# cram9030/continuum-robot

Hardware: AMD Instinct MI355X
Metric: beam-element-steps/s (higher is better)
Workload: dtype f64

## Files before the change

### continuum-robot_amd/csrc/crb_blocked.h

```cpp
#pragma once
#include <cmath>
#include <cstring>
#include <vector>

#include "crb_math.h"

namespace crb {

constexpr int BLK_NPL = 4;
constexpr int BLK_LANES = 64;
constexpr int BLK_S = BLK_NPL * BLK_LANES;
constexpr int BLK_MAX_LV = 6;
constexpr int BLK_PACK = 5;
enum : int {
    BU_L1 = 0, BU_L2 = 5, BU_D0 = 10, BU_D1 = 15, BU_D2 = 20, BU_U0 = 25, BU_U1 = 30,
    BU_WL = 35, BU_WR = 50, BU_AS = 65, BU_CS = 70, BU_N = 76
};
__host__ __device__ constexpr int blk_sep_vals(int levels) { return levels * PCR_LEVEL_VALS + BLK_PACK; }
__host__ __device__ constexpr int blk_fold_offset(int levels) { return BU_N + blk_sep_vals(levels) * BLK_LANES; }

constexpr int BLK_TAB_ROW = 16;
constexpr int BLK_TAB_REGS = (BU_N + BLK_TAB_ROW - 1) / BLK_TAB_ROW;
__host__ __device__ constexpr int blk_tab_index(int reg, int lane) {
    return BLK_TAB_ROW * reg + (lane & (BLK_TAB_ROW - 1)) < BU_N - 1 ? BLK_TAB_ROW * reg + (lane & (BLK_TAB_ROW - 1)) : BU_N - 1;
}

#if defined(__HIPCC__)
template <int OFF, typename T>
__device__ __forceinline__ void blk_bc_fnma(const T (&tab)[BLK_TAB_REGS], T x, T& acc) {
    static_assert(OFF >= 0 && OFF < BU_N, "table offset");
#if defined(__HIP_DEVICE_COMPILE__)
    asm("v_fmac_f64_dpp %0, -%1, %2 row_newbcast:%3 row_mask:0xf bank_mask:0xf"
        : "+v"(acc) : "v"(tab[OFF / BLK_TAB_ROW]), "v"(x), "n"(OFF % BLK_TAB_ROW));
#else
    acc -= tab[OFF / BLK_TAB_ROW] * x;
#endif
}
template <int OFF, typename T>
__device__ __forceinline__ void blk_bc_fma(const T (&tab)[BLK_TAB_REGS], T x, T& acc) {
    static_assert(OFF >= 0 && OFF < BU_N, "table offset");
#if defined(__HIP_DEVICE_COMPILE__)
    asm("v_fmac_f64_dpp %0, %1, %2 row_newbcast:%3 row_mask:0xf bank_mask:0xf"
        : "+v"(acc) : "v"(tab[OFF / BLK_TAB_ROW]), "v"(x), "n"(OFF % BLK_TAB_ROW));
#else
    acc += tab[OFF / BLK_TAB_ROW] * x;
#endif
}
template <int OFF, typename T>
__device__ __forceinline__ T blk_bc_copy(const T (&tab)[BLK_TAB_REGS]) {
    static_assert(OFF >= 0 && OFF < BU_N, "table offset");
#if defined(__HIP_DEVICE_COMPILE__)
    T d;
    asm("v_mov_b64_dpp %0, %1 row_newbcast:%2 row_mask:0xf bank_mask:0xf" : "=v"(d) : "v"(tab[OFF / BLK_TAB_ROW]), "n"(OFF % BLK_TAB_ROW));
    return d;
#else
    return tab[OFF / BLK_TAB_ROW];
#endif
}
template <int OFF, typename T>
__device__ __forceinline__ void blk_bc_sub_mul(const T (&tab)[BLK_TAB_REGS], const T v[3], T o[3]) {
    blk_bc_fnma<OFF + 0>(tab, v[0], o[0]);
    blk_bc_fnma<OFF + 1>(tab, v[1], o[1]);
    blk_bc_fnma<OFF + 2>(tab, v[2], o[1]);
    blk_bc_fnma<OFF + 3>(tab, v[1], o[2]);
    blk_bc_fnma<OFF + 4>(tab, v[2], o[2]);
}
#endif

template <typename T, typename P = const T*>
__host__ __device__ __forceinline__ void blk_mul(P m, const T v[3], T o[3]) {
    o[0] = m[0] * v[0];
    o[1] = m[1] * v[1] + m[2] * v[2];
    o[2] = m[3] * v[1] + m[4] * v[2];
}
template <typename T, typename P = const T*>
__host__ __device__ __forceinline__ void blk_sub_mul(P m, const T v[3], T o[3]) {
    o[0] = o[0] - m[0] * v[0];
    o[1] = o[1] - m[1] * v[1] - m[2] * v[2];
    o[2] = o[2] - m[3] * v[1] - m[4] * v[2];
}
template <typename T, typename P = const T*>
__host__ __device__ __forceinline__ void blk_interior_solve(P u, const T r[][3], T y[3][3]) {
    T z1[3] = {r[1][0], r[1][1], r[1][2]}, z2[3] = {r[2][0], r[2][1], r[2][2]};
    blk_sub_mul<T, P>(u + BU_L1, r[0], z1);
    blk_sub_mul<T, P>(u + BU_L2, z1, z2);
    blk_mul<T, P>(u + BU_D2, z2, y[2]);
    blk_mul<T, P>(u + BU_D1, z1, y[1]);
    blk_sub_mul<T, P>(u + BU_U1, y[2], y[1]);
    blk_mul<T, P>(u + BU_D0, r[0], y[0]);
    blk_sub_mul<T, P>(u + BU_U0, y[1], y[0]);
}

struct Blk2 {
    double ax = 0.0, m[4] = {0.0, 0.0, 0.0, 0.0};
};
inline Blk2 b2_mul(const Blk2& a, const Blk2& b) {
    Blk2 r;
    r.ax = a.ax * b.ax;
    mul2(a.m, b.m, r.m);
    return r;
}
inline Blk2 b2_sub(const Blk2& a, const Blk2& b) {
// ... 159 lines not shown
```

### continuum-robot_amd/csrc/crb_lean.h

```cpp
#pragma once
#include <hip/hip_runtime.h>

#include "crb_blocked.h"
#include "crb_generic.h"

namespace crb {

template <typename T>
struct LeanRec {
    static constexpr int N = sizeof(T) == 8 ? 10 : 12;
    static constexpr int V = 16 / sizeof(T);
};
template <typename T>
__host__ __device__ constexpr size_t lean_lds_bytes(int NT, int lognw) {
    return sizeof(T) * (size_t(NT + 1) * LeanRec<T>::N * (lognw == 1 ? 2 : 1) +
                        (sizeof(T) == 4 ? 4 : 3) * size_t(NT + 1) * size_t(lognw > 1 ? lognw - 1 : 0));
}

__device__ __forceinline__ double dpp_from_lower(double x) {
    int lo = __double2loint(x), hi = __double2hiint(x);
    lo = __builtin_amdgcn_mov_dpp(lo, 0x138, 0xf, 0xf, true);
    hi = __builtin_amdgcn_mov_dpp(hi, 0x138, 0xf, 0xf, true);
    return __hiloint2double(hi, lo);
}
// ... 66 lines not shown
            for (int c = 0; c < 3; ++c) {
                switch (l - LOGNW) {
                    case 0: rlo[c] = lane_lower<T, 1>(r[c], lane); rhi[c] = lane_higher<T, 1>(r[c], lane); break;
                    case 1: rlo[c] = lane_lower<T, 2>(r[c], lane); rhi[c] = lane_higher<T, 2>(r[c], lane); break;
                    case 2: rlo[c] = lane_lower<T, 4>(r[c], lane); rhi[c] = lane_higher<T, 4>(r[c], lane); break;
                    case 3: rlo[c] = lane_lower<T, 8>(r[c], lane); rhi[c] = lane_higher<T, 8>(r[c], lane); break;
                    case 4: rlo[c] = lane_lower<T, 16>(r[c], lane); rhi[c] = lane_higher<T, 16>(r[c], lane); break;
                    default: rlo[c] = lane_lower<T, 32>(r[c], lane); rhi[c] = lane_higher<T, 32>(r[c], lane); break;
                }
            }
            if (ISOLATE) {
                const int st = 1 << l;
                const bool lo_ok = valid && j - st >= 0, hi_ok = valid && j + st < S;
#pragma unroll
                for (int c = 0; c < 3; ++c) { rlo[c] = lo_ok ? rlo[c] : T(0); rhi[c] = hi_ok ? rhi[c] : T(0); }
            }
        }
        pcr_apply_level<T>(cf.lv[l], rlo, rhi, r);
    }
    CRB_SETPRIO(sizeof(T) == 4 ? P32_FIN : P_FIN);
    pcr_apply_final<T>(cf.fin, r, a);
}

template <typename T, int LV, int LOGNW, int EM>
__device__ __forceinline__ void lean_rhs(const ElemCoef<T>& ec, T dragc, bool corrected, const SolveCoef<T, LV>& cf, T* lds3, int t,
                                         int lane, int j, int S, bool valid, const T sq[3], const T sv[3], const T uadd[3], T a[3]) {
    constexpr int NW = 1 << LOGNW, NT = 64 << LOGNW, NULLT = NT;
    T* const ldsQ = lds3;
    T* const ldsA = lds3 + 3 * size_t(NT + 1);
    T* const ldsB = lds3 + 9 * size_t(NT + 1);
    auto thread_of = [](int jj) { return ((jj & (NW - 1)) << 6) | (jj >> LOGNW); };
    const int t_l1 = (valid && j >= 1) ? thread_of(j - 1) : NULLT;
    const int t_r1 = (valid && j + 1 < S) ? thread_of(j + 1) : NULLT;
    const int t_r2 = (valid && j + 2 < S) ? thread_of(j + 2) : NULLT;
    T qL[3];
    if (LOGNW == 0) {
#pragma unroll
        for (int c = 0; c < 3; ++c) qL[c] = lane_lower<T, 1>(sq[c], lane);
    } else {
#pragma unroll
        for (int c = 0; c < 3; ++c) ldsQ[size_t(c) * (NT + 1) + t] = sq[c];
        __syncthreads();
#pragma unroll
        for (int c = 0; c < 3; ++c) qL[c] = ldsQ[size_t(c) * (NT + 1) + t_l1];
    }
    T fl[3], fr[3];
    if (EM == EM_NONLINEAR) elem_force_nonlinear<T>(ec.c, qL, sq, false, fl, fr);
    else if (EM == EM_LINEAR) elem_force_linear<T>(ec.c, qL, sq, fl, fr);
    else elem_force<T>(ec, qL, sq, corrected, fl, fr);
    T pp[3];
#pragma unroll
    for (int c = 0; c < 3; ++c) pp[c] = uadd[c] - fr[c];
    pp[1] += drag_force<T>(dragc, sv[1]);
    T r[3], rlo[3], rhi[3];
    if (LOGNW == 0) {
#pragma unroll
        for (int c = 0; c < 3; ++c) {
            r[c] = pp[c] - lane_higher<T, 1>(fl[c], lane);
            rlo[c] = lane_lower<T, 1>(r[c], lane);
            rhi[c] = lane_higher<T, 1>(r[c], lane);
        }
    } else {
        auto col = [&](int k, int th) -> T& { return ldsA[size_t(k) * (NT + 1) + th]; };
#pragma unroll
        for (int c = 0; c < 3; ++c) { col(c, t) = pp[c]; col(3 + c, t) = fl[c]; }
        __syncthreads();
#pragma unroll
        for (int c = 0; c < 3; ++c) {
            rlo[c] = col(c, t_l1) - fl[c];
            r[c] = pp[c] - col(3 + c, t_r1);
            rhi[c] = col(c, t_r1) - col(3 + c, t_r2);
        }
    }
    pcr_apply_level<T>(cf.lv[0], rlo, rhi, r);
    lean_reduce_tail<T, LV, LOGNW>(cf, ldsB, t, lane, j, S, valid, r, a);
}

#ifndef CRB_BLK_CHORD
#define CRB_BLK_CHORD 1
#endif
#ifndef CRB_BLK_FOLD
#define CRB_BLK_FOLD 1
#endif
#ifndef CRB_BLK_RK4_POS
#define CRB_BLK_RK4_POS 1
#endif
constexpr int BLK_STRIP_PAD = 4;
constexpr int BLK_STRIP_W = BLK_STRIP_PAD + BLK_LANES + BLK_STRIP_PAD;
__host__ __device__ constexpr size_t blk_lds_bytes(int ls) {
    return size_t(blk_sep_vals(ls) + 1) / 2 * 2 * BLK_LANES * sizeof(double) + size_t(4) * 3 * BLK_STRIP_W * sizeof(double);
}
template <typename T, int LS, int EM, typename KPT>
__device__ __forceinline__ void lean_blocked_body(KPT kp) {
    static_assert(sizeof(T) == 8, "the blocked stepper is fp64");
    static_assert(LS == 3 && (1 << (LS - 1)) == BLK_STRIP_PAD, "the strip carries the third separator level, stride 4");
    constexpr int NP = BLK_NPL, NV = blk_sep_vals(LS), NV2 = (NV + 1) / 2;
    constexpr bool REGROUP = EM == EM_NONLINEAR && !CRB_LITERAL_POLY;
    constexpr bool CHORD = CRB_BLK_CHORD, RKPOS = CRB_BLK_RK4_POS;
    constexpr bool FOLD = REGROUP && CRB_BLK_FOLD;
#if defined(__HIP_DEVICE_COMPILE__)
    typedef const __attribute__((address_space(4))) SlotConst<T>* CS;
    typedef const __attribute__((address_space(4))) T* CK;
#define CRB_BFRESH(ptr) asm volatile("" : "+s"(ptr))
#else
    typedef const SlotConst<T>* CS;
    typedef const T* CK;
#define CRB_BFRESH(ptr) (void)(ptr)
#endif
    typedef T rec4 __attribute__((ext_vector_type(4)));
    typedef T pair2 __attribute__((ext_vector_type(2)));
    KParams<T> p = *(const KParams<T>*)(kp);
    extern __shared__ __attribute__((aligned(16))) unsigned char crb_smem[];
    pair2* const sepL = reinterpret_cast<pair2*>(crb_smem);
    T* const strips = reinterpret_cast<T*>(sepL + NV2 * 64);
    const int t = threadIdx.x, lane = t & 63;
    const int wave = __builtin_amdgcn_readfirstlane(t >> 6);
    {
        const T* src = p.blocked + BU_N;
        for (int i = t; i < NV2 * 64; i += 256) {
            const int v = 2 * (i >> 6), l = i & 63;
            sepL[i] = pair2{src[size_t(v) * 64 + l], v + 1 < NV ? src[size_t(v + 1) * 64 + l] : T(0)};
        }
        for (int i = t; i < 4 * 3 * BLK_STRIP_W; i += 256) {
            const int k = i % BLK_STRIP_W;
            if (k < BLK_STRIP_PAD || k >= BLK_STRIP_PAD + BLK_LANES) strips[i] = T(0);
        }
    }
#if defined(__HIP_DEVICE_COMPILE__)
    typedef volatile __attribute__((address_space(3))) T* SP;
#else
    typedef volatile T* SP;
#endif
    const SP strip = (SP)(strips + wave * 3 * BLK_STRIP_W + BLK_STRIP_PAD + lane);
    T tab[BLK_TAB_REGS];
#pragma unroll
    for (int i = 0; i < BLK_TAB_REGS; ++i) tab[i] = p.blocked[blk_tab_index(i, lane)];
    const T cD2[3] = {blk_bc_copy<BU_D2>(tab), blk_bc_copy<BU_D2 + 2>(tab), blk_bc_copy<BU_D2 + 4>(tab)};
    const T cD1[3] = {blk_bc_copy<BU_U1>(tab), blk_bc_copy<BU_D1 + 2>(tab), blk_bc_copy<BU_D1 + 4>(tab)};
    const T cD0[3] = {blk_bc_copy<BU_U0>(tab), blk_bc_copy<BU_D0 + 2>(tab), blk_bc_copy<BU_D0 + 4>(tab)};
    __syncthreads();
    const int n_groups = (p.B + 3) / 4;
    for (int grp = blockIdx.x; grp < n_groups; grp += gridDim.x) {
        CRB_BFRESH(kp);
        p = *(const KParams<T>*)(kp);
        const int beam = grp * 4 + wave;
        if (beam >= p.B) continue;
        const size_t plane = size_t(p.n_node) * 4;
        const size_t xoff = size_t(beam) * 2 * plane + size_t(NP * lane + p.off) * 4;
        T xq[NP][3], xv[NP][3];
#pragma unroll
        for (int k = 0; k < NP; ++k) {
            const rec4 a = *reinterpret_cast<const rec4*>(p.x + xoff + 4 * k), b = *reinterpret_cast<const rec4*>(p.x + xoff + plane + 4 * k);
#pragma unroll
            for (int c = 0; c < 3; ++c) { xq[k][c] = a[c]; xv[k][c] = b[c]; }
        }
        T amp = T(0);
        int kimp = -1;
        if (p.amp) {
            const int js = p.imp_node_b ? p.imp_node_b[beam] - p.off : p.imp_slot;
            if (js >= 0 && js < BLK_S) {
                kimp = js & (NP - 1);
                if (lane == js / NP) amp = p.amp[beam];
            }
        }
        T qL[3];
#pragma unroll
        for (int c = 0; c < 3; ++c) qL[c] = dpp_from_lower(xq[NP - 1][c]);
        const T dt = T(p.dt), hdt = T(0.5 * p.dt), dt6 = T(p.dt / 6.0);
        [[maybe_unused]] const T c6 = T(p.dt * p.dt / 6.0), c4 = T(0.25 * p.dt * p.dt), c2 = T(0.5 * p.dt * p.dt);
        double tc = p.t0;
        [[maybe_unused]] T accq[NP][3], accv[NP][3];
        T sq[NP][3], sv[NP][3];
        [[maybe_unused]] Rk4Pos<T> rk[NP][3];
        for (int step = 0; step < p.n_steps; ++step) {
            double t_half, t_full;
            {
                KPT ks = kp;
                CRB_BFRESH(ks);
                const double hstep = (*(const KParams<T>*)(ks)).dt;
                t_half = __dadd_rn(tc, 0.5 * hstep);
                t_full = __dadd_rn(tc, hstep);
            }
#pragma unroll
            for (int k = 0; k < NP; ++k)
#pragma unroll
                for (int c = 0; c < 3; ++c) { sq[k][c] = xq[k][c]; sv[k][c] = xv[k][c]; }
#pragma unroll
            for (int s = 0; s < 4; ++s) {
                KPT ks = kp;
                CRB_BFRESH(ks);
                const KParams<T>& q = *(const KParams<T>*)(ks);
                const double ts = (s == 0) ? tc : ((s == 3) ? t_full : t_half);
                const bool imp_on = ts < q.duration;
                const T w = (s == 0 || s == 3) ? T(1) : T(2);
                const T cs = (s == 2) ? dt : hdt;
                const CS SC = (CS)q.slot;
                [[maybe_unused]] T ec[6];
                [[maybe_unused]] T fk[FK_N];
                if constexpr (FOLD) {
                    const CK FC = (CK)q.blocked + blk_fold_offset(LS);
#pragma unroll
                    for (int i = 0; i < FK_N; ++i) fk[i] = FC[i];
                } else {
#pragma unroll
                    for (int i = 0; i < 6; ++i) ec[i] = SC->elem.c[i];
                }
                const T drag_all = SC->drag;
                const T dragc = (q.flags & 1u) ? drag_all : T(0);
                [[maybe_unused]] T qn3[3];
                T qLn[3];
                if constexpr (RKPOS) {
                    if (s == 0) {
#pragma unroll
                        for (int k = 0; k < NP; ++k)
#pragma unroll
                            for (int c = 0; c < 3; ++c) rk4_begin<T>(rk[k][c], xq[k][c], xv[k][c], hdt, dt);
                    }
#pragma unroll
                    for (int c = 0; c < 3; ++c) qLn[c] = dpp_from_lower(rk[NP - 1][c].next);
                } else {
#pragma unroll
                    for (int k = 0; k < NP; ++k)
#pragma unroll
                        for (int c = 0; c < 3; ++c) accq[k][c] = (s == 0) ? sv[k][c] : accq[k][c] + w * sv[k][c];
#pragma unroll
                    for (int c = 0; c < 3; ++c) {
                        qn3[c] = (s == 3) ? (xq[NP - 1][c] + dt6 * accq[NP - 1][c]) : (xq[NP - 1][c] + cs * sv[NP - 1][c]);
                        qLn[c] = dpp_from_lower(qn3[c]);
                    }
                }
                CRB_SETPRIO(P_FORCE);
                T fl[NP][3], r[NP][3];
                T fr[NP][3];
                T f2[NP], cW[NP];
#pragma unroll
                for (int k = 0; k < NP; ++k) {
                    if constexpr (FOLD) {
                        const ElemForceRegrouped<T> e = elem_force_nonlinear_folded<T, const T*>(fk, k ? sq[k - 1] : qL, sq[k]);
                        f2[k] = e.f2; cW[k] = e.W;
                        fl[k][1] = e.f3; fr[k][1] = -e.f3; fl[k][2] = e.m_left; fr[k][2] = e.m_right;
                    } else if constexpr (REGROUP) {
                        const ElemForceRegrouped<T> e = CHORD ? elem_force_nonlinear_chord<T>(ec, k ? sq[k - 1] : qL, sq[k])
                                                              : elem_force_nonlinear_regrouped<T>(ec, k ? sq[k - 1] : qL, sq[k]);
                        f2[k] = e.f2; cW[k] = ec[1] * e.W;
                        fl[k][1] = e.f3; fr[k][1] = -e.f3; fl[k][2] = e.m_left; fr[k][2] = e.m_right;
                    } else if (EM == EM_NONLINEAR) elem_force_nonlinear<T>(ec, k ? sq[k - 1] : qL, sq[k], false, fl[k], fr[k]);
                    else elem_force_linear<T>(ec, k ? sq[k - 1] : qL, sq[k], fl[k], fr[k]);
                }
                if constexpr (REGROUP) {
                    fl[0][0] = cW[0] - f2[0];
#pragma unroll
                    for (int k = 0; k + 1 < NP; ++k) fr[k][0] = f2[k] - f2[k + 1];
                    fr[NP - 1][0] = dpp_from_higher(fl[0][0]);
                }
                {
                    const int kon = imp_on ? kimp : -1, dof = q.imp_dof;
#if defined(__HIP_DEVICE_COMPILE__)
#pragma unroll
                    for (int k = 0; k < NP; ++k)
                        asm volatile(
                            "s_cmp_lg_u32 %[kon], %[k]\n\t"
                            "s_cbranch_scc1 2f\n\t"
                            "s_cmp_lg_u32 %[dof], 0\n\t"
                            "s_cbranch_scc1 0f\n\t"
                            "v_add_f64 %[f0], %[f0], -%[amp]\n"
                            "0:\n\t"
                            "s_cmp_lg_u32 %[dof], 1\n\t"
                            "s_cbranch_scc1 1f\n\t"
                            "v_add_f64 %[f1], %[f1], -%[amp]\n"
                            "1:\n\t"
                            "s_cmp_lg_u32 %[dof], 2\n\t"
                            "s_cbranch_scc1 2f\n\t"
                            "v_add_f64 %[f2], %[f2], -%[amp]\n"
                            "2:"
                            : [f0] "+v"(fr[k][0]), [f1] "+v"(fr[k][1]), [f2] "+v"(fr[k][2])
                            : [kon] "s"(kon), [dof] "s"(dof), [amp] "v"(amp), [k] "n"(k)
                            : "scc");
#else
                    for (int k = 0; k < NP; ++k)
                        for (int c = 0; c < 3; ++c) fr[k][c] -= (kon == k && c == dof) ? amp : T(0);
#endif
                }
                CRB_SETPRIO(P_TAIL);
#pragma unroll
                for (int c = 0; c < 3; ++c) {
                    if (REGROUP && c == 0) {
#pragma unroll
                        for (int k = 0; k < NP; ++k) r[k][0] = (k + 1 < NP) ? (-fr[k][0] - cW[k + 1]) : (-f2[k] - fr[k][0]);
                        continue;
                    }
                    const T flR = dpp_from_higher(fl[0][c]);
#pragma unroll
                    for (int k = 0; k < NP; ++k) {
                        T h = -fr[k][c];
                        if (c == 1) h += drag_force<T>(dragc, sv[k][1]);
                        r[k][c] = h - ((k + 1 < NP) ? fl[k + 1][c] : flR);
                    }
                }
                T y[3][3], z1[3], z2[3], g[3], y0R[3];
                int li = lane;
                T cf0[PCR_LEVEL_VALS];
                asm volatile("" : "+v"(li) : "v"(r[0][0]));
#pragma unroll
                for (int i = 0; i < PCR_LEVEL_VALS; i += 2) {
                    const pair2 e = sepL[(i / 2) * 64 + li];
                    cf0[i] = e[0]; cf0[i + 1] = e[1];
                }
#pragma unroll
                for (int c = 0; c < 3; ++c) { z1[c] = r[1][c]; z2[c] = r[2][c]; g[c] = r[NP - 1][c]; }
                blk_bc_sub_mul<BU_L1>(tab, r[0], z1);
                blk_bc_sub_mul<BU_L2>(tab, z1, z2);
                y[2][0] = cD2[0] * z2[0];
                y[2][1] = cD2[1] * z2[2]; blk_bc_fma<BU_D2 + 1>(tab, z2[1], y[2][1]);
                y[2][2] = cD2[2] * z2[2]; blk_bc_fma<BU_D2 + 3>(tab, z2[1], y[2][2]);
                y[1][0] = -(cD1[0] * y[2][0]); blk_bc_fma<BU_D1>(tab, z1[0], y[1][0]);
                y[1][1] = cD1[1] * z1[2]; blk_bc_fma<BU_D1 + 1>(tab, z1[1], y[1][1]);
                y[1][2] = cD1[2] * z1[2]; blk_bc_fma<BU_D1 + 3>(tab, z1[1], y[1][2]);
                blk_bc_fnma<BU_U1 + 1>(tab, y[2][1], y[1][1]); blk_bc_fnma<BU_U1 + 2>(tab, y[2][2], y[1][1]);
                blk_bc_fnma<BU_U1 + 3>(tab, y[2][1], y[1][2]); blk_bc_fnma<BU_U1 + 4>(tab, y[2][2], y[1][2]);
                y[0][0] = -(cD0[0] * y[1][0]); blk_bc_fma<BU_D0>(tab, r[0][0], y[0][0]);
                y[0][1] = cD0[1] * r[0][2]; blk_bc_fma<BU_D0 + 1>(tab, r[0][1], y[0][1]);
                y[0][2] = cD0[2] * r[0][2]; blk_bc_fma<BU_D0 + 3>(tab, r[0][1], y[0][2]);
                blk_bc_fnma<BU_U0 + 1>(tab, y[1][1], y[0][1]); blk_bc_fnma<BU_U0 + 2>(tab, y[1][2], y[0][1]);
                blk_bc_fnma<BU_U0 + 3>(tab, y[1][1], y[0][2]); blk_bc_fnma<BU_U0 + 4>(tab, y[1][2], y[0][2]);
#pragma unroll
                for (int c = 0; c < 3; ++c) y0R[c] = dpp_from_higher(y[0][c]);
                blk_bc_sub_mul<BU_AS>(tab, y[2], g);
                blk_bc_sub_mul<BU_CS>(tab, y0R, g);
#pragma unroll
                for (int l = 0; l < LS; ++l) {
                    asm volatile("" : "+v"(li) : "v"(g[0]));
                    T cf[PCR_LEVEL_VALS];
#pragma unroll
                    for (int i = 0; i < PCR_LEVEL_VALS; i += 2) {
                        const int v = l * PCR_LEVEL_VALS + i;
                        if (l == 0) { cf[i] = cf0[i]; cf[i + 1] = cf0[i + 1]; continue; }
                        const pair2 e = sepL[(v / 2) * 64 + li];
                        cf[i] = e[0]; cf[i + 1] = e[1];
                    }
                    T glo[3], ghi[3];
                    if (l == 2) {
#pragma unroll
                        for (int c = 0; c < 3; ++c) strip[c * BLK_STRIP_W] = g[c];
#pragma unroll
                        for (int c = 0; c < 3; ++c) { glo[c] = strip[c * BLK_STRIP_W - 4]; ghi[c] = strip[c * BLK_STRIP_W + 4]; }
                    } else if (l == 1) {
#pragma unroll
                        for (int c = 0; c < 3; ++c) { glo[c] = lane_lower<T, 2>(g[c], lane); ghi[c] = lane_higher<T, 2>(g[c], lane); }
                    } else {
#pragma unroll
                        for (int c = 0; c < 3; ++c) { glo[c] = lane_lower<T, 1>(g[c], lane); ghi[c] = lane_higher<T, 1>(g[c], lane); }
                    }
                    pcr_apply_level<T>(cf, glo, ghi, g);
                }
                asm volatile("" : "+v"(li) : "v"(g[0]));
                T fin[6], xs[3], xsL[3];
#pragma unroll
                for (int i = 0; i < 6; i += 2) {
                    const int v = LS * PCR_LEVEL_VALS + i;
                    const pair2 e = sepL[(v / 2) * 64 + li];
                    fin[i] = e[0]; fin[i + 1] = e[1];
                }
                pcr_apply_final<T>(fin, g, xs);
#pragma unroll
                for (int c = 0; c < 3; ++c) xsL[c] = dpp_from_lower(xs[c]);
                T a[NP][3];
#pragma unroll
                for (int k = 0; k < NP - 1; ++k)
#pragma unroll
                    for (int c = 0; c < 3; ++c) a[k][c] = y[k][c];
                static_assert(NP == 4, "three interior nodes, written out: the table offsets are template arguments");
                blk_bc_sub_mul<BU_WL>(tab, xsL, a[0]);
                blk_bc_sub_mul<BU_WR>(tab, xs, a[0]);
                blk_bc_sub_mul<BU_WL + BLK_PACK>(tab, xsL, a[1]);
                blk_bc_sub_mul<BU_WR + BLK_PACK>(tab, xs, a[1]);
                blk_bc_sub_mul<BU_WL + 2 * BLK_PACK>(tab, xsL, a[2]);
                blk_bc_sub_mul<BU_WR + 2 * BLK_PACK>(tab, xs, a[2]);
#pragma unroll
                for (int c = 0; c < 3; ++c) a[NP - 1][c] = xs[c];
#pragma unroll
                for (int k = 0; k < NP; ++k)
// ... 680 lines not shown
```

### continuum-robot_amd/csrc/crb_math.h

```cpp
#pragma once
#include <math.h>
#include <stdint.h>

#if defined(__HIPCC__)
#define CRB_HD __host__ __device__ __forceinline__
#else
#define CRB_HD inline
#endif

namespace crb {

enum : int { KIND_NONE = 0, KIND_LINEAR = 1, KIND_NONLINEAR = 2 };

template <typename T>
struct ElemCoef {
    T c[6];
    int32_t kind;
    int32_t pad;
};

template <typename T>
CRB_HD void elem_coef_build(ElemCoef<T>& e, int kind, double L, double E, double I, double A) {
    const double EA = E * A, EI = E * I;
    e.kind = kind;
// ... 214 lines not shown
};
#if defined(__HIPCC__)
__host__
#endif
inline void elem_fold_build(const ElemCoef<double>& e, double k[FK_N]) {
    const long double L = e.c[0], cA1 = e.c[1], cA3 = e.c[2], cD3 = e.c[3], cA4 = e.c[4], cD4 = e.c[5];
    const long double L2 = L * L, L3 = L2 * L;
    k[FK_EPS] = double(2.0L / L);
    k[FK_F2_DW2] = double(cA1 / 2.0L);
    k[FK_F2_DU] = double(-(cA1 * L));
    k[FK_F2_D2] = double(cA1 * L2 / 24.0L);
    k[FK_F2_E2] = double(cA1 * L2 / 40.0L);
    k[FK_LT_0] = double(cA1 * L);
    k[FK_LT_E] = double(cA1 * L / 20.0L);
    k[FK_LT_DW] = double(-(cA1 / 2.0L));
    k[FK_F3E_0] = double(-(3.0L * cD3 * L));
    k[FK_F3E_DU] = double(cA3 * L2);
    k[FK_F3E_D2] = double(3.0L * cA3 * L3 / 56.0L);
    k[FK_F3E_DW2] = double(-(3.0L * cA3 * L / 2.0L));
    k[FK_F3E_E2] = double(-(cA3 * L3 / 56.0L));
    k[FK_F3W_D2] = double(3.0L * cA3 * L2 / 4.0L);
    k[FK_F3W_DU] = double(-(10.0L * cA3 * L));
    k[FK_F3W_DW2] = double(5.0L * cA3);
    k[FK_F3W_E2] = double(15.0L * cA3 * L2 / 28.0L);
    k[FK_XE_0] = double(3.0L * cD4 * L);
    k[FK_XE_D2] = double(11.0L * cA4 * L3 / 560.0L);
    k[FK_XE_DU] = double(-(cA4 * L2 / 10.0L));
    k[FK_XE_DW2] = double(3.0L * cA4 * L / 20.0L);
    k[FK_XE_E2] = double(3.0L * cA4 * L3 / 560.0L);
    k[FK_XW_D2] = double(cA4 * L2 / 20.0L);
    k[FK_XW_E2] = double(3.0L * cA4 * L2 / 140.0L);
    k[FK_R_0] = double(cD4 * L);
    k[FK_R_D2] = double(cA4 * L3 / 80.0L);
    k[FK_R_DU] = double(-(cA4 * L2 / 6.0L));
    k[FK_R_E2] = double(11.0L * cA4 * L3 / 560.0L);
    k[FK_R_DW] = double(cA4 * L / 4.0L);
    k[FK_R_E] = double(cA4 * L2 / 10.0L);
}
template <typename T, typename K = const T*>
CRB_HD ElemForceRegrouped<T> elem_force_nonlinear_folded(K k, const T ql[3], const T qr[3]) {
    const T u2 = qr[0];
    const T du = ql[0] - u2, dw = ql[1] - qr[1];
    const T sg = ql[2] + qr[2], dl = ql[2] - qr[2];
    const T eps = sg - k[FK_EPS] * dw;
    const T e2 = eps * eps, d2 = dl * dl, dw2 = dw * dw;

    T f2 = k[FK_F2_DW2] * dw2;
    f2 = f2 + k[FK_F2_DU] * du;
    f2 = f2 + k[FK_F2_D2] * d2;
    f2 = f2 + k[FK_F2_E2] * e2;
    T LT = k[FK_LT_0] + k[FK_LT_E] * eps;
    LT = LT + k[FK_LT_DW] * dw;

    T F3e = k[FK_F3E_0] + k[FK_F3E_DU] * du;
    F3e = F3e + k[FK_F3E_D2] * d2;
    F3e = F3e + k[FK_F3E_DW2] * dw2;
    F3e = F3e + k[FK_F3E_E2] * e2;
    T F3w = k[FK_F3W_D2] * d2;
    F3w = F3w + k[FK_F3W_DU] * du;
    F3w = F3w + k[FK_F3W_DW2] * dw2;
    F3w = F3w + k[FK_F3W_E2] * e2;
    T Xe = k[FK_XE_0] + k[FK_XE_D2] * d2;
    Xe = Xe + k[FK_XE_DU] * du;
    Xe = Xe + k[FK_XE_DW2] * dw2;
    Xe = Xe + k[FK_XE_E2] * e2;
    const T Xw = k[FK_XW_D2] * d2 + k[FK_XW_E2] * e2;
    const T X = eps * Xe + dw * Xw;
    T Rf = k[FK_R_0] + k[FK_R_D2] * d2;
    Rf = Rf + k[FK_R_DU] * du;
    Rf = Rf + k[FK_R_E2] * e2;
    Rf = Rf + dw * (k[FK_R_DW] * dw + k[FK_R_E] * eps);
    const T Y = dl * Rf;

    ElemForceRegrouped<T> o;
    o.f2 = f2;
    o.W = u2 * LT;
    o.f3 = eps * F3e + dw * F3w;
    o.m_left = X + Y;
    o.m_right = X - Y;
    return o;
}

template <typename T>
struct Rk4Pos {
    T next;
    T full;
    T sum;
    T accv;
};
template <typename T>
CRB_HD void rk4_begin(Rk4Pos<T>& r, T q, T v, T hdt, T dt) {
    r.next = q + hdt * v;
    r.full = q + dt * v;
}
template <typename T>
CRB_HD void rk4_end0(Rk4Pos<T>& r, T a, T c6, T c4) {
    r.accv = a;
    r.sum = r.full + c6 * a;
    r.next = r.next + c4 * a;
}
template <typename T>
CRB_HD void rk4_end1(Rk4Pos<T>& r, T a, T c6, T c2) {
    r.accv = r.accv + T(2) * a;
    r.sum = r.sum + c6 * a;
    r.full = r.full + c2 * a;
    r.next = r.full;
}
template <typename T>
CRB_HD void rk4_end2(Rk4Pos<T>& r, T a, T c6) {
    r.accv = r.accv + T(2) * a;
    r.next = r.sum + c6 * a;
}
template <typename T>
CRB_HD T rk4_end3(const Rk4Pos<T>& r, T v, T a, T dt6) {
    return v + dt6 * (r.accv + a);
}
template <typename T>
CRB_HD T rk4_stage_velocity(T v, T cs, T a) {
    return v + cs * a;
}

#ifndef CRB_LITERAL_POLY
#define CRB_LITERAL_POLY 0
#endif
template <typename T>
CRB_HD void elem_force_nonlinear(const T* c, const T ql[3], const T qr[3], bool corrected, T fl[3], T fr[3]) {
#if CRB_LITERAL_POLY
    const T iL2 = T(1) / (c[0] * c[0]);
    const T lit[5] = {c[0], c[1] / iL2, c[5] / iL2, iL2, T(0.1) * iL2 / c[0]};
    elem_force_nonlinear_literal<T>(lit, ql, qr, corrected, fl, fr);
#else
    elem_force_nonlinear_sym<T>(c, ql, qr, corrected, fl, fr);
#endif
}

template <typename T>
CRB_HD void elem_force(const ElemCoef<T>& e, const T ql[3], const T qr[3], bool corrected, T fl[3], T fr[3]) {
    if (e.kind == KIND_NONLINEAR) {
        elem_force_nonlinear<T>(e.c, ql, qr, corrected, fl, fr);
    } else if (e.kind == KIND_LINEAR) {
        elem_force_linear<T>(e.c, ql, qr, fl, fr);
    } else {
        fl[0] = fl[1] = fl[2] = fr[0] = fr[1] = fr[2] = T(0);
    }
}

CRB_HD void crb_sincos(double x, double* s, double* c) {
#if defined(__HIP_DEVICE_COMPILE__)
    ::sincos(x, s, c);
#else
    *s = sin(x);
    *c = cos(x);
#endif
}
CRB_HD void crb_sincos(float x, float* s, float* c) {
#if defined(__HIP_DEVICE_COMPILE__)
    ::sincosf(x, s, c);
#else
    *s = sinf(x);
    *c = cosf(x);
#endif
}

template <typename T>
CRB_HD void gravity_segment(T phi, T gx, T gy, T half_mass, T out[2]) {
    T s, c;
// ... 291 lines not shown
```

### continuum-robot_amd/csrc/crbeam.hip

```cpp
#include <hip/hip_runtime.h>

#include <cmath>
#include <cstdio>
#include <cstdlib>
#include <cstring>
#include <ctime>
#include <string>
#include <type_traits>
#include <vector>

#include "../../include/crbeam.h"
#include "crb_kernels.h"
#include "crb_lean_launch.h"
#include "crb_loop_launch.h"
#include "crb_ctrl_launch.h"
#include "crb_static_launch.h"
#include "crb_tangent_launch.h"
#include "crb_adjoint_launch.h"
#include "crb_feedback_adjoint_launch.h"
#include "crb_host.h"
#include "crb_blocked.h"

using namespace crb;

// ... 223 lines not shown
        for (int r = 0; r < n; ++r) {
            const int f = r < int(p->free_index.size()) ? p->free_index[r] : 0;
            row[r] = (f / 3) * 4 + (f % 3);
            col[r] = row[r];
            col[n + r] = p->n_node * 4 + row[r];
        }
        HIP_TRY(hipMalloc(reinterpret_cast<void**>(&p->d_col_off), col.size() * sizeof(int32_t)));
        HIP_TRY(hipMalloc(reinterpret_cast<void**>(&p->d_row_off), row.size() * sizeof(int32_t)));
        HIP_TRY(hipMemcpy(p->d_col_off, col.data(), col.size() * sizeof(int32_t), hipMemcpyHostToDevice));
        HIP_TRY(hipMemcpy(p->d_row_off, row.data(), row.size() * sizeof(int32_t), hipMemcpyHostToDevice));
    }
    if (nd > 1) {
        p->slot_stride = size_t(S);
        p->lv_stride = size_t(lf) * S * PCR_LEVEL_VALS;
        p->fin_stride = size_t(S) * PCR_FINAL_VALS;
    }

    AsmParams a;
    std::memset(&a, 0, sizeof(a));
    a.L = dL.p; a.E = dE.p; a.I = dI.p; a.rho = dRho.p; a.A = dA.p;
    a.nonlinear = dNl.p; a.free_dof = dFree.p; a.wet = dWet.p; a.cd = dCd.p; a.grav = dGrav.p;
    a.fluid_density = d->fluid_density; a.flags = d->flags;
    a.n_elem = ne; a.n_node = p->n_node; a.off = p->off; a.S = S; a.levels_full = lf;
    if (nd > 1) { a.n_elem_b = dNe.p; a.fluid_density_b = dFd.p; a.flags_b = dFl.p; }
    a.free_stride = per_beam_topo ? size_t(nn) * 3 : 0;
    a.grav_stride = per_beam_topo ? size_t(S) : 0;
    a.slot_out = p->d_slot; a.lv64 = dLv64.p; a.lvT = p->d_levels; a.fin64_all = dFinAll.p; a.norms = dNorms.p;
    a.blocks0 = dBlocks.p; a.finT = nullptr; a.fin_level = -1;
    a.elem_stride = nd > 1 ? size_t(ne) : 0;
    const int nta = (S + 63) / 64 * 64;
    const size_t smem = size_t(S) * sizeof(NodeBlocks);
    HIP_TRY(lds_opt_in(crb_assemble_kernel<T>, smem));
    HIP_TRY(hipMemset(dNorms.p, 0, size_t(lf ? lf : 1) * sizeof(double)));
    hipLaunchKernelGGL((crb_assemble_kernel<T>), dim3(nd), dim3(nta), smem, nullptr, a);
    HIP_TRY(hipGetLastError());
    HIP_TRY(hipDeviceSynchronize());
    p->h_levels.assign(size_t(lf > 0 ? lf : 1) * S * PCR_LEVEL_VALS, 0.0);
    p->h_norms.assign(size_t(lf > 0 ? lf : 1), 0.0);
    if (lf > 0) {
        HIP_TRY(hipMemcpy(p->h_levels.data(), dLv64.p, size_t(lf) * S * PCR_LEVEL_VALS * sizeof(double), hipMemcpyDeviceToHost));
        HIP_TRY(hipMemcpy(p->h_norms.data(), dNorms.p, size_t(lf) * sizeof(double), hipMemcpyDeviceToHost));
    }
    const int used = pick_levels(p);
    if (used > MAX_LV)
        return fail(CRB_EUNSUPPORTED, "mass matrix needs more cyclic-reduction levels than the kernels carry in registers");
    in.a = a; in.nd = nd; in.threads = nta; in.smem = smem;
    a.finT = p->d_final; a.fin_level = used; a.lv64 = nullptr; a.blocks0 = nullptr; a.fin64_all = nullptr;
    hipLaunchKernelGGL((crb_assemble_kernel<T>), dim3(nd), dim3(nta), smem, nullptr, a);
    HIP_TRY(hipGetLastError());
    HIP_TRY(hipDeviceSynchronize());

    p->h_final.assign(size_t(S) * PCR_FINAL_VALS, 0.0);
    HIP_TRY(hipMemcpy(p->h_final.data(), dFinAll.p + size_t(used) * S * PCR_FINAL_VALS,
                      size_t(S) * PCR_FINAL_VALS * sizeof(double), hipMemcpyDeviceToHost));
    std::vector<double> b0(size_t(S) * 15);
    HIP_TRY(hipMemcpy(b0.data(), dBlocks.p, b0.size() * sizeof(double), hipMemcpyDeviceToHost));
    std::vector<NodeBlocks> blk(S);
    for (int j = 0; j < S; ++j) {
        const double* b = &b0[size_t(j) * 15];
        blk[j].a_ax = b[0]; blk[j].b_ax = b[1]; blk[j].c_ax = b[2];
        for (int k = 0; k < 4; ++k) { blk[j].A[k] = b[3 + k]; blk[j].B[k] = b[7 + k]; blk[j].C[k] = b[11 + k]; }
    }
    mass_from_blocks(p, blk);
    std::vector<SlotConst<T>> hs(S);
    HIP_TRY(hipMemcpy(hs.data(), p->d_slot, size_t(S) * sizeof(SlotConst<T>), hipMemcpyDeviceToHost));
    p->h_slots.assign(S, SlotConst<double>());
    p->h_kinds.assign(S, KIND_NONE);
    for (int j = 0; j < S; ++j) {
        SlotConst<double>& o = p->h_slots[j];
        std::memset(&o, 0, sizeof(o));
        o.drag = double(hs[j].drag);
        o.half_mass = double(hs[j].half_mass);
        for (int c = 0; c < 3; ++c) o.mask[c] = double(hs[j].mask[c]);
        o.grav = hs[j].grav;
        p->h_kinds[j] = hs[j].elem.kind;
    }
    if constexpr (sizeof(T) == 8) {
        bool uniform = nd == 1 && S == BLK_S && p->G == 1;
        for (int j = 0; uniform && j < S; ++j)
            uniform = std::memcmp(&hs[j].elem, &hs[0].elem, sizeof(hs[0].elem)) == 0 &&
                      std::memcmp(&hs[j].drag, &hs[0].drag, sizeof(T)) == 0 && hs[j].mask[0] == T(1) && hs[j].mask[1] == T(1) &&
                      hs[j].mask[2] == T(1);
        if (uniform) {
            std::vector<double> tab(size_t(blk_fold_offset(BLK_MAX_LV)) + FK_N);
            double norms[BLK_MAX_LV];
            const int lv = blocked_factor(blk.data(), d->length[0], tab.data(), tab.data() + BU_N, norms);
            if (lv >= 1) {
                const bool fold = hs[0].elem.kind == KIND_NONLINEAR;
                const size_t n = size_t(blk_fold_offset(lv)) + (fold ? FK_N : 0);
                if (fold) {
                    ElemCoef<double> ecd;
                    for (int i = 0; i < 6; ++i) ecd.c[i] = double(hs[0].elem.c[i]);
                    elem_fold_build(ecd, tab.data() + blk_fold_offset(lv));
                }
                HIP_TRY(hipMalloc(reinterpret_cast<void**>(&p->d_blocked), n * sizeof(double)));
                HIP_TRY(hipMemcpy(p->d_blocked, tab.data(), n * sizeof(double), hipMemcpyHostToDevice));
                p->blocked_levels = lv;
            }
        }
    }
    return CRB_OK;
}

}

static int plan_create_impl(crb_plan** out, int device, int dtype, int n_beams, const crb_beam_desc* d, int nd);

extern "C" int crb_plan_create(crb_plan** out, int device, int dtype, int n_beams, const crb_beam_desc* d) {
    return plan_create_impl(out, device, dtype, n_beams, d, 1);
}

extern "C" int crb_plan_create_ensemble(crb_plan** out, int device, int dtype, int n_beams, const crb_beam_desc* descs) {
    if (!out || !descs) return fail(CRB_EINVAL, "crb_plan_create_ensemble: null argument");
    if (n_beams < 1) return fail(CRB_EINVAL, "n_beams must be >= 1");
    if (device < 0) return fail(CRB_EUNSUPPORTED, "per-beam coefficient plans are built on the device (no host-only form)");
    const crb_beam_desc& a = descs[0];
    for (int b = 1; b < n_beams; ++b)
        if ((descs[b].flags & CRB_CORRECTED_AXIAL) != (a.flags & CRB_CORRECTED_AXIAL))
            return fail(CRB_EINVAL, "ensemble beams must share the CRB_CORRECTED_AXIAL option");
    return plan_create_impl(out, device, dtype, n_beams, descs, n_beams);
}

namespace {
const char* validate_desc(const crb_beam_desc& o) {
    if (o.n_elem < 1) return "n_elem must be >= 1";
    if (!o.length || !o.elastic_modulus || !o.moment_inertia || !o.density || !o.cross_area || !o.nonlinear || !o.node_bc)
        return "beam description has null columns";
    for (int e = 0; e < o.n_elem; ++e) {
        if (!(o.length[e] > 0) || !(o.elastic_modulus[e] > 0) || !(o.moment_inertia[e] > 0) || !(o.density[e] > 0) ||
            !(o.cross_area[e] > 0))
            return "All numeric parameters must be positive";
        if (o.nonlinear[e] > 1) return "Invalid element type";
    }
    for (int i = 0; i <= o.n_elem; ++i)
        if (o.node_bc[i] != CRB_BC_NONE && o.node_bc[i] != CRB_BC_FIXED && o.node_bc[i] != CRB_BC_PINNED)
            return "Unsupported boundary condition type";
    if (o.flags & CRB_FORCE_DRAG) {
        if (!o.wetted_area || !o.drag_coef) return "drag enabled but wetted_area/drag_coef missing";
        if (!(o.fluid_density > 0)) return "fluid_density must be positive when fluid effects are enabled";
        for (int e = 0; e < o.n_elem; ++e) {
            if (o.drag_coef[e] < 0) return "Drag coefficients cannot be negative";
            if (o.wetted_area[e] < 0) return "Wetted areas cannot be negative";
        }
    }
    return nullptr;
}

BeamTopo build_topology(const crb_beam_desc& d, int nn, int off) {
    BeamTopo t;
    const int ne = d.n_elem, S = nn - off;
    t.n_elem = ne;
    t.free_dof.assign(size_t(nn) * 3, 0);
    for (int i = 0; i <= ne; ++i) {
        const int bc = d.node_bc[i];
        const bool fx = bc == CRB_BC_FIXED, pin = bc == CRB_BC_PINNED;
        t.free_dof[3 * i] = t.free_dof[3 * i + 1] = (fx || pin) ? 0 : 1;
        t.free_dof[3 * i + 2] = fx ? 0 : 1;
    }
    t.full2red.assign(size_t(nn) * 3, -1);
    for (int f = 0; f < 3 * nn; ++f)
        if (t.free_dof[f]) { t.full2red[f] = int32_t(t.free_index.size()); t.free_index.push_back(f); }
    t.n_free = int(t.free_index.size());
    const int n = t.n_free;
    t.grav.resize(S);
    const bool grav = d.flags & CRB_FORCE_GRAVITY;
    for (int j = 0; j < S; ++j) {
        GravTab& gt = t.grav[j];
        gt.phiA = gt.phiB = -1;
        for (int c = 0; c < 3; ++c) { gt.segA[c] = gt.segB[c] = -1; gt.comp[c] = 0; }
        gt.pad = 0;
        if (!grav) continue;
        const int node = j + off;
        auto enc = [&](int red) -> int16_t {
            const int f = t.free_index[red];
            return int16_t(((f / 3) - off) * 4 + (f % 3));
        };
// ... 2337 lines not shown
```

Baseline: 78.82 billion.

## Share subexpressions in folded element force and prefetch constants across stages

Adds a host-built table of coefficients that lets the nonlinear element force reuse common terms (A1/A2, dw*eps), so each element needs fewer flops. The force constants are now loaded once before the loop and re-loaded for the next stage after the residual is formed, hiding scalar-load latency. Duration, impulse dof and drag are also held in registers instead of being re-read every stage. The cost is extra SGPR pressure, slightly different rounding from the regrouped arithmetic, and inline-asm ordering constraints.

New measurement: 82.70 billion, median of 6. 1.05x the previous value.

```diff
diff --git a/continuum-robot_amd/csrc/crb_blocked.h b/continuum-robot_amd/csrc/crb_blocked.h
--- a/continuum-robot_amd/csrc/crb_blocked.h
+++ b/continuum-robot_amd/csrc/crb_blocked.h
@@ -18,6 +18,7 @@
 };
 __host__ __device__ constexpr int blk_sep_vals(int levels) { return levels * PCR_LEVEL_VALS + BLK_PACK; }
 __host__ __device__ constexpr int blk_fold_offset(int levels) { return BU_N + blk_sep_vals(levels) * BLK_LANES; }
+__host__ __device__ constexpr int blk_share_offset(int levels) { return blk_fold_offset(levels) + FK_N; }
 
 constexpr int BLK_TAB_ROW = 16;
 constexpr int BLK_TAB_REGS = (BU_N + BLK_TAB_ROW - 1) / BLK_TAB_ROW;
diff --git a/continuum-robot_amd/csrc/crb_lean.h b/continuum-robot_amd/csrc/crb_lean.h
--- a/continuum-robot_amd/csrc/crb_lean.h
+++ b/continuum-robot_amd/csrc/crb_lean.h
@@ -172,6 +172,15 @@
 #ifndef CRB_BLK_FOLD
 #define CRB_BLK_FOLD 1
 #endif
+#ifndef CRB_BLK_SHARE
+#define CRB_BLK_SHARE 1
+#endif
+#ifndef CRB_BLK_CONST_AHEAD
+#define CRB_BLK_CONST_AHEAD 1
+#endif
+#ifndef CRB_BLK_HOLD_PARAMS
+#define CRB_BLK_HOLD_PARAMS 1
+#endif
 #ifndef CRB_BLK_RK4_POS
 #define CRB_BLK_RK4_POS 1
 #endif
@@ -188,6 +197,10 @@
     constexpr bool REGROUP = EM == EM_NONLINEAR && !CRB_LITERAL_POLY;
     constexpr bool CHORD = CRB_BLK_CHORD, RKPOS = CRB_BLK_RK4_POS;
     constexpr bool FOLD = REGROUP && CRB_BLK_FOLD;
+    constexpr bool SHARE = FOLD && CRB_BLK_SHARE;
+    constexpr int NK = SHARE ? int(SK_N) : int(FK_N);
+    constexpr bool AHEAD = FOLD && CRB_BLK_CONST_AHEAD;
+    constexpr bool HOLD = AHEAD && CRB_BLK_HOLD_PARAMS;
 #if defined(__HIP_DEVICE_COMPILE__)
     typedef const __attribute__((address_space(4))) SlotConst<T>* CS;
     typedef const __attribute__((address_space(4))) T* CK;
@@ -262,6 +275,23 @@
         [[maybe_unused]] T accq[NP][3], accv[NP][3];
         T sq[NP][3], sv[NP][3];
         [[maybe_unused]] Rk4Pos<T> rk[NP][3];
+        [[maybe_unused]] T fk_ahead[NK];
+        [[maybe_unused]] CK FC_held = nullptr;
+        [[maybe_unused]] double dur_held = 0.0;
+        [[maybe_unused]] int dof_held = 0;
+        [[maybe_unused]] T dragc_held = T(0);
+        if constexpr (AHEAD) {
+            const CK FC = (CK)p.blocked + (SHARE ? blk_share_offset(LS) : blk_fold_offset(LS));
+#pragma unroll
+            for (int i = 0; i < NK; ++i) fk_ahead[i] = FC[i];
+            if constexpr (HOLD) {
+                FC_held = FC;
+                dur_held = p.duration;
+                dof_held = p.imp_dof;
+                const T drag_all = ((CS)p.slot)->drag;
+                dragc_held = (p.flags & 1u) ? drag_all : T(0);
+            }
+        }
         for (int step = 0; step < p.n_steps; ++step) {
             double t_half, t_full;
             {
@@ -281,22 +311,27 @@
                 CRB_BFRESH(ks);
                 const KParams<T>& q = *(const KParams<T>*)(ks);
                 const double ts = (s == 0) ? tc : ((s == 3) ? t_full : t_half);
-                const bool imp_on = ts < q.duration;
+                const bool imp_on = ts < (HOLD ? dur_held : q.duration);
                 const T w = (s == 0 || s == 3) ? T(1) : T(2);
                 const T cs = (s == 2) ? dt : hdt;
                 const CS SC = (CS)q.slot;
                 [[maybe_unused]] T ec[6];
-                [[maybe_unused]] T fk[FK_N];
+                [[maybe_unused]] T fk_stage[NK];
+                [[maybe_unused]] T* const fk = AHEAD ? fk_ahead : fk_stage;
+                [[maybe_unused]] CK FCn = nullptr;
                 if constexpr (FOLD) {
-                    const CK FC = (CK)q.blocked + blk_fold_offset(LS);
-#pragma unroll
-                    for (int i = 0; i < FK_N; ++i) fk[i] = FC[i];
+                    const CK FC = (CK)q.blocked + (SHARE ? blk_share_offset(LS) : blk_fold_offset(LS));
+                    if constexpr (AHEAD) FCn = HOLD ? FC_held : FC;
+                    else {
+#pragma unroll
+                        for (int i = 0; i < NK; ++i) fk[i] = FC[i];
+                    }
                 } else {
 #pragma unroll
                     for (int i = 0; i < 6; ++i) ec[i] = SC->elem.c[i];
                 }
                 const T drag_all = SC->drag;
-                const T dragc = (q.flags & 1u) ? drag_all : T(0);
+                const T dragc = HOLD ? dragc_held : ((q.flags & 1u) ? drag_all : T(0));
                 [[maybe_unused]] T qn3[3];
                 T qLn[3];
                 if constexpr (RKPOS) {
@@ -326,7 +361,9 @@
 #pragma unroll
                 for (int k = 0; k < NP; ++k) {
                     if constexpr (FOLD) {
-                        const ElemForceRegrouped<T> e = elem_force_nonlinear_folded<T, const T*>(fk, k ? sq[k - 1] : qL, sq[k]);
+                        ElemForceRegrouped<T> e;
+                        if constexpr (SHARE) e = elem_force_nonlinear_shared<T, const T*>(fk, k ? sq[k - 1] : qL, sq[k]);
+                        else e = elem_force_nonlinear_folded<T, const T*>(fk, k ? sq[k - 1] : qL, sq[k]);
                         f2[k] = e.f2; cW[k] = e.W;
                         fl[k][1] = e.f3; fr[k][1] = -e.f3; fl[k][2] = e.m_left; fr[k][2] = e.m_right;
                     } else if constexpr (REGROUP) {
@@ -344,7 +381,7 @@
                     fr[NP - 1][0] = dpp_from_higher(fl[0][0]);
                 }
                 {
-                    const int kon = imp_on ? kimp : -1, dof = q.imp_dof;
+                    const int kon = imp_on ? kimp : -1, dof = HOLD ? dof_held : q.imp_dof;
 #if defined(__HIP_DEVICE_COMPILE__)
 #pragma unroll
                     for (int k = 0; k < NP; ++k)
@@ -387,6 +424,15 @@
                         r[k][c] = h - ((k + 1 < NP) ? fl[k + 1][c] : flR);
                     }
                 }
+                if constexpr (AHEAD) {
+#if defined(__HIP_DEVICE_COMPILE__)
+                    asm volatile("" : "+s"(FCn)
+                                 : "v"(r[0][0]), "v"(r[0][1]), "v"(r[0][2]), "v"(r[1][0]), "v"(r[1][1]), "v"(r[1][2]),
+                                   "v"(r[2][0]), "v"(r[2][1]), "v"(r[2][2]), "v"(r[3][0]), "v"(r[3][1]), "v"(r[3][2]));
+#endif
+#pragma unroll
+                    for (int i = 0; i < NK; ++i) fk_ahead[i] = FCn[i];
+                }
                 T y[3][3], z1[3], z2[3], g[3], y0R[3];
                 int li = lane;
                 T cf0[PCR_LEVEL_VALS];
diff --git a/continuum-robot_amd/csrc/crb_math.h b/continuum-robot_amd/csrc/crb_math.h
--- a/continuum-robot_amd/csrc/crb_math.h
+++ b/continuum-robot_amd/csrc/crb_math.h
@@ -320,6 +320,96 @@
 }
 
 template <typename T>
+CRB_HD T fused_madd(T a, T b, T c);
+template <>
+CRB_HD double fused_madd<double>(double a, double b, double c) { return __builtin_fma(a, b, c); }
+template <>
+CRB_HD float fused_madd<float>(float a, float b, float c) { return __builtin_fmaf(a, b, c); }
+enum : int {
+    SK_EPS = 0, SK_A1, SK_A2,
+    SK_F2_A, SK_F2_D2, SK_F2_E2,
+    SK_LT_0, SK_LT_E, SK_LT_DW,
+    SK_F3E_0, SK_F3E_A, SK_F3E_D2, SK_F3E_E2,
+    SK_F3W_A, SK_F3W_D2, SK_F3W_E2,
+    SK_XE_0, SK_XE_A, SK_XE_D2, SK_XE_E2,
+    SK_XW_D2, SK_XW_E2,
+    SK_R_0, SK_R_A, SK_R_D2, SK_R_E2, SK_R_DWE,
+    SK_N
+};
+#if defined(__HIPCC__)
+__host__
+#endif
+inline void elem_share_build(const ElemCoef<double>& e, double k[SK_N]) {
+    const long double L = e.c[0], cA1 = e.c[1], cA3 = e.c[2], cD3 = e.c[3], cA4 = e.c[4], cD4 = e.c[5];
+    const long double L2 = L * L, L3 = L2 * L;
+    k[SK_EPS] = double(2.0L / L);
+    k[SK_A1] = double(-(2.0L * L));
+    k[SK_A2] = double(-(2.0L * L / 3.0L));
+    k[SK_F2_A] = double(cA1 / 2.0L);
+    k[SK_F2_D2] = double(cA1 * L2 / 24.0L);
+    k[SK_F2_E2] = double(cA1 * L2 / 40.0L);
+    k[SK_LT_0] = double(cA1 * L);
+    k[SK_LT_E] = double(cA1 * L / 20.0L);
+    k[SK_LT_DW] = double(-(cA1 / 2.0L));
+    k[SK_F3E_0] = double(-(3.0L * cD3 * L));
+    k[SK_F3E_A] = double(-(3.0L * cA3 * L / 2.0L));
+    k[SK_F3E_D2] = double(3.0L * cA3 * L3 / 56.0L);
+    k[SK_F3E_E2] = double(-(cA3 * L3 / 56.0L));
+    k[SK_F3W_A] = double(5.0L * cA3);
+    k[SK_F3W_D2] = double(3.0L * cA3 * L2 / 4.0L);
+    k[SK_F3W_E2] = double(15.0L * cA3 * L2 / 28.0L);
+    k[SK_XE_0] = double(3.0L * cD4 * L);
+    k[SK_XE_A] = double(3.0L * cA4 * L / 20.0L);
+    k[SK_XE_D2] = double(11.0L * cA4 * L3 / 560.0L);
+    k[SK_XE_E2] = double(3.0L * cA4 * L3 / 560.0L);
+    k[SK_XW_D2] = double(cA4 * L2 / 20.0L);
+    k[SK_XW_E2] = double(3.0L * cA4 * L2 / 140.0L);
+    k[SK_R_0] = double(cD4 * L);
+    k[SK_R_A] = double(cA4 * L / 4.0L);
+    k[SK_R_D2] = double(cA4 * L3 / 80.0L);
+    k[SK_R_E2] = double(11.0L * cA4 * L3 / 560.0L);
+    k[SK_R_DWE] = double(cA4 * L2 / 10.0L);
+}
+template <typename T, typename K = const T*>
+CRB_HD ElemForceRegrouped<T> elem_force_nonlinear_shared(K k, const T ql[3], const T qr[3]) {
+    const T u2 = qr[0];
+    const T du = ql[0] - u2, dw = ql[1] - qr[1];
+    const T sg = ql[2] + qr[2], dl = ql[2] - qr[2];
+    const T eps = sg - k[SK_EPS] * dw;
+    const T e2 = eps * eps, d2 = dl * dl, dw2 = dw * dw;
+    const T A1 = dw2 + k[SK_A1] * du, A2 = dw2 + k[SK_A2] * du;
+
+    T f2 = fused_madd<T>(k[SK_F2_D2], d2, k[SK_F2_A] * A1);
+    f2 = f2 + k[SK_F2_E2] * e2;
+    T LT = k[SK_LT_0] + k[SK_LT_E] * eps;
+    LT = LT + k[SK_LT_DW] * dw;
+
+    T F3e = k[SK_F3E_0] + k[SK_F3E_A] * A2;
+    F3e = F3e + k[SK_F3E_D2] * d2;
+    F3e = F3e + k[SK_F3E_E2] * e2;
+    T F3w = fused_madd<T>(k[SK_F3W_D2], d2, k[SK_F3W_A] * A1);
+    F3w = F3w + k[SK_F3W_E2] * e2;
+    T Xe = k[SK_XE_0] + k[SK_XE_A] * A2;
+    Xe = Xe + k[SK_XE_D2] * d2;
+    Xe = Xe + k[SK_XE_E2] * e2;
+    const T Xw = fused_madd<T>(k[SK_XW_E2], e2, k[SK_XW_D2] * d2);
+    const T X = fused_madd<T>(dw, Xw, eps * Xe);
+    T Rf = k[SK_R_0] + k[SK_R_A] * A2;
+    Rf = Rf + k[SK_R_D2] * d2;
+    Rf = Rf + k[SK_R_E2] * e2;
+    Rf = Rf + k[SK_R_DWE] * (dw * eps);
+    const T Y = dl * Rf;
+
+    ElemForceRegrouped<T> o;
+    o.f2 = f2;
+    o.W = u2 * LT;
+    o.f3 = fused_madd<T>(dw, F3w, eps * F3e);
+    o.m_left = X + Y;
+    o.m_right = X - Y;
+    return o;
+}
+
+template <typename T>
 struct Rk4Pos {
     T next;
     T full;
diff --git a/continuum-robot_amd/csrc/crbeam.hip b/continuum-robot_amd/csrc/crbeam.hip
--- a/continuum-robot_amd/csrc/crbeam.hip
+++ b/continuum-robot_amd/csrc/crbeam.hip
@@ -329,16 +329,17 @@
                       std::memcmp(&hs[j].drag, &hs[0].drag, sizeof(T)) == 0 && hs[j].mask[0] == T(1) && hs[j].mask[1] == T(1) &&
                       hs[j].mask[2] == T(1);
         if (uniform) {
-            std::vector<double> tab(size_t(blk_fold_offset(BLK_MAX_LV)) + FK_N);
+            std::vector<double> tab(size_t(blk_share_offset(BLK_MAX_LV)) + SK_N);
             double norms[BLK_MAX_LV];
             const int lv = blocked_factor(blk.data(), d->length[0], tab.data(), tab.data() + BU_N, norms);
             if (lv >= 1) {
                 const bool fold = hs[0].elem.kind == KIND_NONLINEAR;
-                const size_t n = size_t(blk_fold_offset(lv)) + (fold ? FK_N : 0);
+                const size_t n = fold ? size_t(blk_share_offset(lv)) + SK_N : size_t(blk_fold_offset(lv));
                 if (fold) {
                     ElemCoef<double> ecd;
                     for (int i = 0; i < 6; ++i) ecd.c[i] = double(hs[0].elem.c[i]);
                     elem_fold_build(ecd, tab.data() + blk_fold_offset(lv));
+                    elem_share_build(ecd, tab.data() + blk_share_offset(lv));
                 }
                 HIP_TRY(hipMalloc(reinterpret_cast<void**>(&p->d_blocked), n * sizeof(double)));
                 HIP_TRY(hipMemcpy(p->d_blocked, tab.data(), n * sizeof(double), hipMemcpyHostToDevice));
```
